# ZhaozhiQIAN/Hybrid-ODE-NeurIPS-2021

Hardware: AMD Instinct MI355X
Metric: patient-trajectories/sec (fwd+adjoint) at dim=12, T=100 (higher is better)
Workload: dtype f32; 1 GPU; dim12 synthetic, 10000 patients/GPU, T=100, dt=0.125, rk4(3/8), fused rhs+step kernel + discrete-adjoint kernel (split expert/learned wave pipelines); patients_total=10000, launch=hipGraph, lanes_per_patient=auto, theta_grad=True, parallelism=dp1, n_ranks=1, stage_tape=True

## Files before the change

### hybrid-ode-neurips-2021_amd/csrc/hode_rk_split.hip

```cpp
#include <hip/hip_runtime.h>
#include <stdlib.h>

#include "../../include/hode.h"
#include "hode_common.hpp"
#include "hode_host.hpp"
#include "hode_roche.hpp"

namespace hode {

#ifndef HODE_SPLIT_EXPERT_FIRST
#define HODE_SPLIT_EXPERT_FIRST 1
#endif
constexpr int kSplitPatients = 48;

struct SplitArgs {
  const float* __restrict__ t;
  const float* __restrict__ y0;
  const float* __restrict__ dosage;
  const float* __restrict__ dose_times;
  const float* __restrict__ theta;
  const float* __restrict__ w1;
  const float* __restrict__ b1;
  float* __restrict__ h;
  float* __restrict__ tape;
  unsigned long long* dbg;
  float* __restrict__ ltape;
  int* __restrict__ status;
  int B, T, K, perturb;
};

struct SpTimes {
  float t0, t1, dt, ts[4];
  HODE_DEV SpTimes(const float* __restrict__ t, int n, int perturb, int method) {
    t0 = t[n];
    t1 = t[n + 1];
    dt = t1 - t0;
    ts[0] = perturb ? nextafter_up(t0) : t0;
    ts[3] = perturb ? nextafter_down(t1) : t1;
    if (method == HODE_METHOD_RK4_38) {
      ts[1] = add_rn(t0, mul_rn(dt, (float)(1.0 / 3.0)));
      ts[2] = add_rn(t0, mul_rn(dt, (float)(2.0 / 3.0)));
    } else {
      ts[1] = add_rn(t0, mul_rn(0.5f, dt));
      ts[2] = ts[1];
    }
  }
};

template <int METHOD>
HODE_DEV float sp_stage_time(float t0, float t1, int perturb, int q) {
  const float dt = t1 - t0;
  const float c = METHOD == HODE_METHOD_RK4_38 ? (q == 1 ? (float)(1.0 / 3.0) : (q == 2 ? (float)(2.0 / 3.0) : 0.f))
                                               : (q == 0 ? 0.f : 0.5f);
  float tq = add_rn(t0, mul_rn(dt, c));
  tq = q == 3 ? t1 : tq;
  if (perturb) {
    if (q == 0) tq = nextafter_up(t0);
    if (q == 3) tq = nextafter_down(t1);
  }
  return tq;
}

constexpr int kSplitMaxT = 8192;
HODE_DEV void sp_stage_grid(float* __restrict__ tg, const float* __restrict__ t, int T) {
  for (int i = threadIdx.x; i < T + 3; i += blockDim.x) tg[i] = t[min(i, T - 1)];
}

template <int METHOD>
constexpr int sp_stages() { return METHOD == HODE_METHOD_EULER ? 1 : (METHOD == HODE_METHOD_MIDPOINT ? 2 : 4); }

template <int METHOD, class V>
HODE_DEV V sp_stage_state(int i, V y, float dt, V k1, V k2, V k3) {
  constexpr float c13 = (float)(1.0 / 3.0);
  if constexpr (METHOD == HODE_METHOD_MIDPOINT) return i == 0 ? y : vfma(k1, vsplat<V>(0.5f * dt), y);
  else if constexpr (METHOD == HODE_METHOD_RK4_38) {
    if (i == 0) return y;
    if (i == 1) return vfma(dt * k1, vsplat<V>(c13), y);
    if (i == 2) return vfma(vsplat<V>(dt), vfma(-k1, vsplat<V>(c13), k2), y);
    return vfma(vsplat<V>(dt), (k1 - k2) + k3, y);
  } else return y;
}
template <int METHOD, class V>
HODE_DEV V sp_advance(V y, float dt, V k1, V k2, V k3, V k4) {
  if constexpr (METHOD == HODE_METHOD_EULER) return vfma(vsplat<V>(dt), k1, y);
  else if constexpr (METHOD == HODE_METHOD_MIDPOINT) return vfma(vsplat<V>(dt), k2, y);
  else return vfma((k1 + 3.0f * (k2 + k3)) + k4, vsplat<V>(dt * 0.125f), y);
}

template <int V> struct IC { static constexpr int value = V; };

template <int MR> struct OwnSel { typedef float type; };
template <> struct OwnSel<2> { typedef f2 type; };

template <bool C, class A, class B> struct TypeSel { typedef A type; };
template <class A, class B> struct TypeSel<false, A, B> { typedef B type; };

#ifndef HODE_LTAPE_STAGES
#define HODE_LTAPE_STAGES 2
#endif
constexpr int kLearnedTapeStages = HODE_LTAPE_STAGES;
template <int METHOD> constexpr int sp_ltape_stages() { return METHOD == HODE_METHOD_RK4_38 ? kLearnedTapeStages : 0; }

template <int D>
struct MlRows {
  static constexpr int M = D - 4, MR = M / 4, DP = D / 2, MP = M / 2;
  static constexpr int NW = MR == 2 ? D : DP;
  static constexpr int NU = MR == 2 ? M : MP;
  static constexpr float kTanhScale = 2.885390081777927f;
  typedef typename OwnSel<MR>::type Own;
  typedef typename TypeSel<MR == 2, float, f2>::type Elem;
  struct Stage { Elem v[NW]; };
  struct Gath { Elem v[NU]; };
  f2 wp[NW];
  Own bias;
  HODE_DEV void load(const float* __restrict__ W, const float* __restrict__ b, int q) {
    if constexpr (MR == 2) {
#pragma unroll
      for (int i = 0; i < D; ++i) wp[i] = kTanhScale * pair2(W[(2 * q) * D + i], W[(2 * q + 1) * D + i]);
      bias = kTanhScale * pair2(b[2 * q], b[2 * q + 1]);
    } else {
#pragma unroll
      for (int ip = 0; ip < DP; ++ip) wp[ip] = kTanhScale * pair2(W[q * D + 2 * ip], W[q * D + 2 * ip + 1]);
      bias = kTanhScale * b[q];
    }
  }
  static HODE_DEV void gather(Own v, Elem* __restrict__ out) {
    if constexpr (MR == 2) {
      out[0] = quad_bcast<0>(v.x); out[1] = quad_bcast<0>(v.y);
      out[2] = quad_bcast<1>(v.x); out[3] = quad_bcast<1>(v.y);
      out[4] = quad_bcast<2>(v.x); out[5] = quad_bcast<2>(v.y);
      out[6] = quad_bcast<3>(v.x); out[7] = quad_bcast<3>(v.y);
    } else {
      out[0] = pair2(quad_bcast<0>(v), quad_bcast<1>(v));
      out[1] = pair2(quad_bcast<2>(v), quad_bcast<3>(v));
    }
  }
  static HODE_DEV Stage stage(const float4& e, Own Yo) {
    Stage Y;
    if constexpr (MR == 2) {
      Y.v[0] = e.x; Y.v[1] = e.y; Y.v[2] = e.z; Y.v[3] = e.w;
      gather(Yo, Y.v + 4);
    } else {
      Y.v[0] = pair2(e.x, e.y);
      Y.v[1] = pair2(e.z, e.w);
      gather(Yo, Y.v + 2);
    }
    return Y;
  }
  static HODE_DEV Own tanh_scaled(Own z) {
    if constexpr (MR == 2) {
      const f2 e = pair2(__builtin_amdgcn_exp2f(z.x), __builtin_amdgcn_exp2f(z.y)) + splat2(1.0f);
      return vfma(pair2(__builtin_amdgcn_rcpf(e.x), __builtin_amdgcn_rcpf(e.y)), splat2(-2.0f), splat2(1.0f));
    } else {
      return __builtin_fmaf(__builtin_amdgcn_rcpf(__builtin_amdgcn_exp2f(z) + 1.0f), -2.0f, 1.0f);
    }
  }
  HODE_DEV Own rhs(const Stage& Y) const {
    if constexpr (MR == 2) {
      f2 acc = bias, acc1 = splat2(0.f);
#pragma unroll
      for (int i = 0; i < D; i += 2) {
        acc = vfma(wp[i], Y.v[i], acc);
        acc1 = vfma(wp[i + 1], Y.v[i + 1], acc1);
      }
      return tanh_scaled(acc + acc1);
    } else {
      f2 acc = pair2(bias, 0.f);
#pragma unroll
      for (int ip = 0; ip < DP; ++ip) acc = vfma(wp[ip], Y.v[ip], acc);
      return tanh_scaled(hsum(acc));
    }
  }
  struct Part { f2 a, b; };
  HODE_DEV Part rhs_expert(const float4& e) const {
    Part p;
    if constexpr (MR == 2) {
      p.a = vfma(wp[2], e.z, vfma(wp[0], e.x, bias));
      p.b = vfma(wp[3], e.w, vfma(wp[1], e.y, splat2(0.f)));
    } else {
      p.a = vfma(wp[1], pair2(e.z, e.w), vfma(wp[0], pair2(e.x, e.y), pair2(bias, 0.f)));
      p.b = splat2(0.f);
    }
    return p;
  }
  HODE_DEV Own rhs_rest(const Part& p, const Stage& Y) const {
    if constexpr (MR == 2) {
      f2 acc = p.a, acc1 = p.b;
#pragma unroll
      for (int i = 4; i < D; i += 2) {
        acc = vfma(wp[i], Y.v[i], acc);
        acc1 = vfma(wp[i + 1], Y.v[i + 1], acc1);
      }
      return tanh_scaled(acc + acc1);
    } else {
      f2 acc = p.a;
#pragma unroll
      for (int ip = 2; ip < DP; ++ip) acc = vfma(wp[ip], Y.v[ip], acc);
      return tanh_scaled(hsum(acc));
    }
  }
  static HODE_DEV void outer_acc(f2 (&dw)[NW], Own u, const Stage& Y) {
#pragma unroll
    for (int i = 0; i < NW; ++i) dw[i] = vfma(u, Y.v[i], dw[i]);
  }
  static HODE_DEV float dw_at(const f2 (&dw)[NW], int r, int i) {
    if constexpr (MR == 2) return r == 0 ? dw[i].x : dw[i].y;
    else return (i & 1) ? dw[i / 2].y : dw[i / 2].x;
  }
  static HODE_DEV Own load_own(const float* __restrict__ src, int q) {
    if constexpr (MR == 2) {
      const float2 x = *reinterpret_cast<const float2*>(src + 4 + 2 * q);
      return pair2(x.x, x.y);
    } else return src[4 + q];
  }
  static HODE_DEV void store_own(float* __restrict__ dst, int q, Own v) {
    if constexpr (MR == 2) *reinterpret_cast<float2*>(dst + 4 + 2 * q) = make_float2(v.x, v.y);
    else dst[4 + q] = v;
  }
  template <int NL>
  static HODE_DEV void store_tape(float* __restrict__ dst, const Own* __restrict__ k) {
    if constexpr (MR == 2 && NL % 2 == 0) {
#pragma unroll
      for (int i = 0; i < NL; i += 2)
        *reinterpret_cast<float4*>(dst + 4 * (i / 2)) = make_float4(k[i].x, k[i].y, k[i + 1].x, k[i + 1].y);
    } else if constexpr (MR == 1 && NL == 4) {
      *reinterpret_cast<float4*>(dst) = make_float4(k[0], k[1], k[2], k[3]);
    } else if constexpr (MR == 1 && NL == 2) {
      *reinterpret_cast<float2*>(dst) = make_float2(k[0], k[1]);
    } else {
#pragma unroll
      for (int i = 0; i < NL; ++i) {
        if constexpr (MR == 2) *reinterpret_cast<float2*>(dst + 2 * i) = make_float2(k[i].x, k[i].y);
        else dst[i] = k[i];
      }
    }
  }
  template <int NL>
  static HODE_DEV void load_tape(const float* __restrict__ src, Own* __restrict__ k) {
    if constexpr (MR == 2 && NL % 2 == 0) {
#pragma unroll
      for (int i = 0; i < NL; i += 2) {
        const float4 v = *reinterpret_cast<const float4*>(src + 4 * (i / 2));
        k[i] = pair2(v.x, v.y); k[i + 1] = pair2(v.z, v.w);
      }
    } else if constexpr (MR == 1 && NL == 4) {
      const float4 v = *reinterpret_cast<const float4*>(src);
      k[0] = v.x; k[1] = v.y; k[2] = v.z; k[3] = v.w;
    } else if constexpr (MR == 1 && NL == 2) {
      const float2 v = *reinterpret_cast<const float2*>(src);
      k[0] = v.x; k[1] = v.y;
    } else {
#pragma unroll
      for (int i = 0; i < NL; ++i) {
        if constexpr (MR == 2) { const float2 v = *reinterpret_cast<const float2*>(src + 2 * i); k[i] = pair2(v.x, v.y); }
        else k[i] = src[i];
      }
    }
  }
};

template <int D, int METHOD, bool ABLATE, bool HILL2, bool K1, bool TAPE>
HODE_DEV void split_fwd_body(const SplitArgs& a) {
  constexpr int NS = sp_stages<METHOD>();
  typedef MlRows<D> Ml;
  typedef typename Ml::Own Own;
  constexpr int DP = Ml::DP;
  __shared__ __attribute__((aligned(16))) float ring[2][4][kSplitPatients][4];
  __shared__ __attribute__((aligned(16))) float dring[2][kSplitPatients][4];
  extern __shared__ float tg[];
  const int tid = threadIdx.x;
  const int wave = tid >> 6, lane = tid & 63;
  const int b0 = blockIdx.x * kSplitPatients;
  const RocheTheta th = load_theta(a.theta, ABLATE);
  const size_t row = (size_t)a.B * D;
  sp_stage_grid(tg, a.t, a.T);
#ifdef HODE_SPLIT_STAMPS
#define HODE_FSTAMP(k) if (a.dbg && blockIdx.x == 0 && lane == 0) a.dbg[(size_t)wave * a.T + (k)] = __builtin_amdgcn_s_memtime();
#else
#define HODE_FSTAMP(k)
#endif

  if (wave == 0) {
    const int slot = lane;
    const bool live = slot < kSplitPatients && b0 + slot < a.B;
    const int p = min(b0 + (slot < kSplitPatients ? slot : 0), a.B - 1);
    const int rslot = slot < kSplitPatients ? slot : 0;
    const unsigned lane_h = (unsigned)p * D, lane_t = (unsigned)p * 4;
    MlSlice<4, 1> none;
    float own1[1];
    f2 ya, yb;
    {
      const float4 v = *reinterpret_cast<const float4*>(a.y0 + (size_t)p * D);
      ya = pair2(v.x, v.y);
      yb = pair2(v.z, v.w);
      if (live) *reinterpret_cast<float4*>(a.h + (size_t)p * D) = v;
    }
    __syncthreads();
    auto e_iter = [&](int it, auto PAR) {
      constexpr int par = decltype(PAR)::value;
      if (it + 1 < a.T) {
        const float dt = tg[it + 1] - tg[it];
        const float4 dz = *reinterpret_cast<const float4*>(&dring[par][rslot][0]);
        const float dose[4] = {dz.x, dz.y, dz.z, dz.w};
        float* __restrict__ tape_it = TAPE ? a.tape + (size_t)it * (NS - 1) * a.B * 4 : nullptr;
        f2 ka[4], kb[4];
#pragma unroll
        for (int s = 0; s < 4; ++s) ka[s] = kb[s] = splat2(0.f);
#pragma unroll
        for (int s = 0; s < NS; ++s) {
          const f2 Ya = sp_stage_state<METHOD>(s, ya, dt, ka[0], ka[1], ka[2]);
          const f2 Yb = sp_stage_state<METHOD>(s, yb, dt, kb[0], kb[1], kb[2]);
          if (slot < kSplitPatients) *reinterpret_cast<float4*>(&ring[par][s][slot][0]) = make_float4(Ya.x, Ya.y, Yb.x, Yb.y);
          if constexpr (TAPE) {
            if (s >= 1)
              *reinterpret_cast<float4*>(tape_it + ((unsigned)(s - 1) * (unsigned)a.B * 4u + lane_t)) = make_float4(Ya.x, Ya.y, Yb.x, Yb.y);
          }
          const float Y[4] = {Ya.x, Ya.y, Yb.x, Yb.y};
          float k[4];
          roche_rhs<4, 1, ABLATE, HILL2>(th, none, dose[s], Y, k, own1);
          ka[s] = pair2(k[0], k[1]);
          kb[s] = pair2(k[2], k[3]);
        }
        ya = sp_advance<METHOD>(ya, dt, ka[0], ka[1], ka[2], ka[3]);
        yb = sp_advance<METHOD>(yb, dt, kb[0], kb[1], kb[2], kb[3]);
        *reinterpret_cast<float4*>(a.h + (size_t)(it + 1) * row + lane_h) = make_float4(ya.x, ya.y, yb.x, yb.y);
      }
      HODE_FSTAMP(it)
      __syncthreads();
    };
    for (int it = 0; it < a.T; it += 2) {
      e_iter(it, IC<0>{});
      if (it + 1 < a.T) e_iter(it + 1, IC<1>{});
    }
    if (a.status) {
      const bool bad = !(vfinite(ya) && vfinite(yb));
      if (bad && live) atomicOr(a.status, HODE_STATUS_NONFINITE);
    }
  } else {
    const int q = lane & 3;
    const int slot = (wave - 1) * 16 + (lane >> 2);
    const bool live = b0 + slot < a.B;
    const int p = min(b0 + slot, a.B - 1);
    Ml ml;
    ml.load(a.w1, a.b1, q);
    DoseSched<K1> ds;
    ds.dosage = a.dosage[p];
    ds.K = a.K;
    ds.taus = a.dose_times + (size_t)p * a.K;
    ds.tau0 = K1 ? ds.taus[0] : 0.f;
    auto dose_step = [&](int parity, float t0, float t1) {
      dring[parity][slot][q] = ds.at(sp_stage_time<METHOD>(t0, t1, a.perturb, q), th.kel).v;
    };
    if (a.T >= 2) dose_step(0, a.t[0], a.t[1]);
    if (a.T >= 3) dose_step(1, a.t[1], a.t[2]);
    Own yo = Ml::load_own(a.y0 + (size_t)p * D, q);
    if (live) Ml::store_own(a.h + (size_t)p * D, q, yo);
    constexpr int NLT = sp_ltape_stages<METHOD>();
    const size_t lt_step = (size_t)a.B * 4 * NLT * Ml::MR;
    const unsigned lt_lane = ((unsigned)p * 4 + q) * NLT * Ml::MR;
    __syncthreads();
    __syncthreads();
    auto m_iter = [&](int it, auto PAR) {
      constexpr int par = decltype(PAR)::value;
      const int n = it - 1;
      const float t_a = tg[it - 1], t_b = tg[it], t_c = tg[it + 1], t_d = tg[it + 2];
      const float dt = t_b - t_a;
      Own k[4];
      float4 e[4];
#pragma unroll
      for (int s = 0; s < NS; ++s) e[s] = *reinterpret_cast<const float4*>(&ring[par][s][slot][0]);
      __builtin_amdgcn_sched_barrier(0);
      dose_step(par, t_c, t_d);
#if HODE_SPLIT_EXPERT_FIRST
      typename Ml::Part pe[4];
#pragma unroll
      for (int s = 0; s < NS; ++s) pe[s] = ml.rhs_expert(e[s]);
#endif
#pragma unroll
      for (int s = 0; s < 4; ++s) k[s] = vsplat<Own>(0.f);
#pragma unroll
      for (int s = 0; s < NS; ++s) {
        const Own Yo = sp_stage_state<METHOD>(s, yo, dt, k[0], k[1], k[2]);
#if HODE_SPLIT_EXPERT_FIRST
        k[s] = ml.rhs_rest(pe[s], Ml::stage(e[s], Yo));
#else
        k[s] = ml.rhs(Ml::stage(e[s], Yo));
#endif
      }
      yo = sp_advance<METHOD>(yo, dt, k[0], k[1], k[2], k[3]);
      Ml::store_own(a.h + (size_t)(n + 1) * row + (size_t)p * D, q, yo);
      if constexpr (TAPE && NLT > 0) Ml::template store_tape<NLT>(a.ltape + (size_t)n * lt_step + lt_lane, k + (NS - NLT));
      HODE_FSTAMP(it)
      __syncthreads();
    };
    for (int it = 1; it < a.T; it += 2) {
      m_iter(it, IC<0>{});
      if (it + 1 < a.T) m_iter(it + 1, IC<1>{});
    }
    if (a.status) {
      if (!vfinite(yo) && live) atomicOr(a.status, HODE_STATUS_NONFINITE);
    }
  }
}

struct SplitBwdArgs {
  const float* __restrict__ t;
  const float* __restrict__ dosage;
  const float* __restrict__ dose_times;
  const float* __restrict__ theta;
  const float* __restrict__ w1;
  const float* __restrict__ b1;
  const float* __restrict__ h;
  const float* __restrict__ grad_h;
  float* __restrict__ grad_y0;
  float* __restrict__ part_ml;
  float* __restrict__ part_th;
  const float* __restrict__ tape;
  const float* __restrict__ ltape;
  int B, T, K, perturb;
  unsigned long long* dbg;
};

template <int METHOD, class V, class F>
HODE_DEV void sp_adjoint_step(V& lam, float dt, F&& vjp) {
  constexpr float c13 = (float)(1.0 / 3.0);
  if constexpr (METHOD == HODE_METHOD_EULER) {
    lam += vjp(0, dt * lam);
  } else if constexpr (METHOD == HODE_METHOD_MIDPOINT) {
    const V a1 = vjp(1, dt * lam);
    lam += a1;
    lam += vjp(0, (0.5f * dt) * a1);
  } else {
    const float w1 = dt * 0.125f, w3 = dt * 0.375f;
    const V a3 = vjp(3, w1 * lam);
    V da = dt * a3;
    V g1 = vfma(w1, lam, da);
    V g2 = vfma(w3, lam, -da);
    const V g = vfma(w3, lam, da);
    lam += a3;
    const V a2 = vjp(2, g);
    da = dt * a2;
    g2 += da;
    g1 = vfma(-c13, da, g1);
    lam += a2;
    const V a1 = vjp(1, g2);
    g1 = vfma(c13, dt * a1, g1);
    lam += a1;
    lam += vjp(0, g1);
  }
}

struct F4 {
  f2 a, b;
  HODE_DEV F4& operator+=(const F4& o) { a += o.a; b += o.b; return *this; }
  HODE_DEV F4 operator-() const { return F4{-a, -b}; }
};
HODE_DEV F4 operator*(float s, const F4& v) { return F4{s * v.a, s * v.b}; }
HODE_DEV F4 vfma(float s, const F4& x, const F4& y) { return F4{vfma(s, x.a, y.a), vfma(s, x.b, y.b)}; }

template <int D, bool CW>
struct SplitBwdShared {
  static constexpr int RD = CW ? 3 : 2;
  static constexpr int M = D - 4;
  float yring[RD][4][kSplitPatients][4];
  float cring[RD][4][kSplitPatients + 1][4];
  float dring[RD][kSplitPatients][8];
  float gring[RD][4][kSplitPatients + 1][4];
  float tdring[RD][kSplitPatients][8];
  float uring[CW ? RD : 1][4][CW ? kSplitPatients : 1][CW ? M : 1];
  float red[4][4][M * D + M];
};

template <int D, int METHOD, bool ABLATE, bool HILL2, bool NEED_TH, bool K1, bool TAPE>
HODE_DEV void split_bwd_body(const SplitBwdArgs& a, SplitBwdShared<D, TAPE>& sh) {
  constexpr int NS = sp_stages<METHOD>();
  typedef MlRows<D> Ml;
  typedef typename Ml::Own Own;
  constexpr int M = Ml::M, MR = Ml::MR, DP = Ml::DP, MP = Ml::MP;
  constexpr bool THW = TAPE && NEED_TH;
  constexpr bool CW = TAPE;
  constexpr int RD = SplitBwdShared<D, TAPE>::RD;
  constexpr int EL = CW ? 2 : 1;
  constexpr int CWAVE = THW ? 5 : 4;
  auto& yring = sh.yring; auto& cring = sh.cring; auto& dring = sh.dring; auto& gring = sh.gring;
  auto& tdring = sh.tdring; auto& uring = sh.uring; auto& red = sh.red;
  extern __shared__ float tg[];
  const int tid = threadIdx.x;
  const int wave = tid >> 6, lane = tid & 63;
  const int b0 = blockIdx.x * kSplitPatients;
  const RocheTheta th = load_theta(a.theta, ABLATE);
  const size_t row = (size_t)a.B * D;
  const int T = a.T;
  const int NIT = T + EL - 1;
  sp_stage_grid(tg, a.t, a.T);
#ifdef HODE_SPLIT_STAMPS
#define HODE_SSTAMP(k) if (a.dbg && blockIdx.x == 0 && lane == 0) a.dbg[(size_t)wave * (a.T + 2) + (k)] = __builtin_amdgcn_s_memtime();
#define HODE_PSTAMP(k, ph) { __builtin_amdgcn_sched_barrier(0); if (a.dbg && blockIdx.x == 0 && wave == 3 && lane == 0) a.dbg[(size_t)6 * (a.T + 2) + 64 + (size_t)(k) * 8 + (ph)] = __builtin_amdgcn_s_memtime(); __builtin_amdgcn_sched_barrier(0); }
  if (a.dbg && blockIdx.x < 8 && lane == 0) a.dbg[(size_t)6 * (a.T + 2) + blockIdx.x * 8 + wave] = __builtin_amdgcn_s_getreg(63492);
#else
#define HODE_SSTAMP(k)
#define HODE_PSTAMP(k, ph)
#endif
  auto run = [&](auto&& iter) {
    for (int k = 0; k < NIT; k += RD) {
      iter(k, IC<0>{});
      if (k + 1 < NIT) iter(k + 1, IC<1>{});
      if constexpr (RD == 3) {
        if (k + 2 < NIT) iter(k + 2, IC<2>{});
      }
    }
  };

  if (wave == 0) {
    const int slot = lane < kSplitPatients ? lane : 0;
    const bool mine = lane < kSplitPatients;
    const bool live = mine && b0 + slot < a.B;
    const int p = min(b0 + slot, a.B - 1);
    const float lv = live ? 1.0f : 0.0f;
    DoseSched<K1> ds;
    ds.dosage = a.dosage[p];
    ds.K = a.K;
    ds.taus = a.dose_times + (size_t)p * a.K;
    ds.tau0 = K1 ? ds.taus[0] : 0.f;
    const float ln_ec50 = log_f32(th.ec50);
    const int cslot = mine ? lane : kSplitPatients;
    if (lane < 16 * RD) (&cring[lane >> 4][(lane >> 2) & 3][kSplitPatients][0])[lane & 3] = 0.f;
    const unsigned lane_h = (unsigned)p * D, lane_t = (unsigned)p * 4;
    MlSlice<4, 1> none;
    MlColSlice<4, 1> nonec;
    GradAcc<4, 1> acc;
    acc.zero();
    float own1[1] = {0.f};

    float tp[4][4];
    auto fetch = [&](int m) {
      const float4 v = *reinterpret_cast<const float4*>(a.h + (size_t)m * row + lane_h);
      tp[0][0] = v.x; tp[0][1] = v.y; tp[0][2] = v.z; tp[0][3] = v.w;
      if constexpr (TAPE) {
        const float* __restrict__ tape_m = a.tape + (size_t)m * (NS - 1) * a.B * 4;
#pragma unroll
        for (int s = 1; s < NS; ++s) {
          const float4 u = *reinterpret_cast<const float4*>(tape_m + ((unsigned)(s - 1) * (unsigned)a.B * 4u + lane_t));
          tp[s][0] = u.x; tp[s][1] = u.y; tp[s][2] = u.z; tp[s][3] = u.w;
        }
      }
    };
    auto publish = [&](int m, int par) {
      if constexpr (TAPE) {
        if (mine) {
#pragma unroll
          for (int s = 0; s < NS; ++s)
            *reinterpret_cast<float4*>(&yring[par][s][slot][0]) = make_float4(tp[s][0], tp[s][1], tp[s][2], tp[s][3]);
        }
      } else {
        const SpTimes st(a.t, m, a.perturb, METHOD);
        const f2 ya = pair2(tp[0][0], tp[0][1]), yb = pair2(tp[0][2], tp[0][3]);
        f2 ka[4], kb[4];
#pragma unroll
        for (int s = 0; s < 4; ++s) ka[s] = kb[s] = splat2(0.f);
#pragma unroll
        for (int s = 0; s < NS; ++s) {
          const f2 Ya = sp_stage_state<METHOD>(s, ya, st.dt, ka[0], ka[1], ka[2]);
          const f2 Yb = sp_stage_state<METHOD>(s, yb, st.dt, kb[0], kb[1], kb[2]);
          const DoseVal dv = ds.at(st.ts[s], th.kel);
          if (mine) {
            *reinterpret_cast<float4*>(&yring[par][s][slot][0]) = make_float4(Ya.x, Ya.y, Yb.x, Yb.y);
            dring[par][slot][s] = dv.v;
            dring[par][slot][4 + s] = dv.dk;
          }
          if (s + 1 < NS) {
            const float Y[4] = {Ya.x, Ya.y, Yb.x, Yb.y};
            float k[4];
            roche_rhs<4, 1, ABLATE, HILL2>(th, none, dv.v, Y, k, own1);
            ka[s] = pair2(k[0], k[1]);
            kb[s] = pair2(k[2], k[3]);
          }
        }
      }
    };

    F4 lam;
    {
      const float4 g4 = *reinterpret_cast<const float4*>(a.grad_h + (size_t)(T - 1) * row + (size_t)p * D);
      lam.a = lv * pair2(g4.x, g4.y);
      lam.b = lv * pair2(g4.z, g4.w);
    }
    if (T >= 2) {
      fetch(T - 2);
      publish(T - 2, 0);
    }
    __syncthreads();
    auto e_iter = [&](int k, auto SI) {
      constexpr int S = decltype(SI)::value;
      constexpr int par = (S + 1) % RD;
      if (T - 3 - k >= 0) fetch(T - 3 - k);
      if (k >= EL && k <= T + EL - 2) {
        const int m = T - k + EL - 2;
        const float dt = tg[m + 1] - tg[m];
        float Y[4][4];
        F4 cs[4];
        DoseVal dv[4];
        {
          const float4 d0 = *reinterpret_cast<const float4*>(&dring[par][slot][0]);
          const float4 d1 = *reinterpret_cast<const float4*>(&dring[par][slot][4]);
          dv[0].v = d0.x; dv[1].v = d0.y; dv[2].v = d0.z; dv[3].v = d0.w;
          dv[0].dk = d1.x; dv[1].dk = d1.y; dv[2].dk = d1.z; dv[3].dk = d1.w;
          if constexpr (THW) {
            *reinterpret_cast<float4*>(&tdring[S][slot][0]) = d0;
            *reinterpret_cast<float4*>(&tdring[S][slot][4]) = d1;
          }
        }
#pragma unroll
        for (int s = 0; s < NS; ++s) {
          const float4 yv = *reinterpret_cast<const float4*>(&yring[par][s][slot][0]);
          const float4 cv = *reinterpret_cast<const float4*>(&cring[par][s][cslot][0]);
          Y[s][0] = yv.x; Y[s][1] = yv.y; Y[s][2] = yv.z; Y[s][3] = yv.w;
          cs[s].a = pair2(cv.x, cv.y);
          cs[s].b = pair2(cv.z, cv.w);
        }
        sp_adjoint_step<METHOD>(lam, dt, [&](int s, const F4& gs) {
          const float g[4] = {gs.a.x, gs.a.y, gs.b.x, gs.b.y};
          float av[4];
          if constexpr (THW) {
            if (mine) *reinterpret_cast<float4*>(&gring[S][s][slot][0]) = make_float4(g[0], g[1], g[2], g[3]);
          }
          roche_vjp<4, 1, ABLATE, HILL2, NEED_TH && !THW>(th, none, nonec, ln_ec50, dv[s], Y[s], own1, g, 0, av, acc);
          F4 r = cs[s];
          r.a += pair2(av[0], av[1]);
          r.b += pair2(av[2], av[3]);
          return r;
        });
        const float4 g4 = *reinterpret_cast<const float4*>(a.grad_h + (size_t)m * row + lane_h);
        lam.a = vfma(lv, pair2(g4.x, g4.y), lam.a);
        lam.b = vfma(lv, pair2(g4.z, g4.w), lam.b);
      }
      if (T - 3 - k >= 0) publish(T - 3 - k, par);
      HODE_SSTAMP(k)
      __syncthreads();
    };
    run(e_iter);
    if (live) *reinterpret_cast<float4*>(a.grad_y0 + (size_t)p * D) = make_float4(lam.a.x, lam.a.y, lam.b.x, lam.b.y);
    if constexpr (!THW) {
#pragma unroll
      for (int i = 0; i < kNTheta; ++i) {
        const float v = row_sum(NEED_TH ? acc.dth[i] : 0.f);
        if ((lane & 15) == 0) red[0][lane >> 4][i] = v;
      }
      __builtin_amdgcn_fence(__ATOMIC_SEQ_CST, "wavefront");
      if (lane < kNTheta)
        a.part_th[(size_t)blockIdx.x * kNTheta + lane] = (red[0][0][lane] + red[0][1][lane]) + (red[0][2][lane] + red[0][3][lane]);
    }
  } else if (THW && wave == 4) {
    const int slot = lane < kSplitPatients ? lane : 0;
    const bool mine = lane < kSplitPatients;
    const int p = min(b0 + slot, a.B - 1);
    const int gslot = mine ? lane : kSplitPatients;
    const float ln_ec50 = log_f32(th.ec50);
    if (lane < 16 * RD) (&gring[lane >> 4][(lane >> 2) & 3][kSplitPatients][0])[lane & 3] = 0.f;
    const unsigned lane_h = (unsigned)p * D, lane_t = (unsigned)p * 4;
    float dth[kNTheta];
#pragma unroll
    for (int i = 0; i < kNTheta; ++i) dth[i] = 0.f;
    float tp[4][4];
    auto fetch = [&](int m) {
      const float4 v = *reinterpret_cast<const float4*>(a.h + (size_t)m * row + lane_h);
      tp[0][0] = v.x; tp[0][1] = v.y; tp[0][2] = v.z; tp[0][3] = v.w;
      const float* __restrict__ tape_m = a.tape + (size_t)m * (NS - 1) * a.B * 4;
#pragma unroll
      for (int s = 1; s < NS; ++s) {
        const float4 u = *reinterpret_cast<const float4*>(tape_m + ((unsigned)(s - 1) * (unsigned)a.B * 4u + lane_t));
        tp[s][0] = u.x; tp[s][1] = u.y; tp[s][2] = u.z; tp[s][3] = u.w;
      }
    };
    auto theta_step = [&](int gpar) {
      const float4 d0 = *reinterpret_cast<const float4*>(&tdring[gpar][slot][0]);
      const float4 d1 = *reinterpret_cast<const float4*>(&tdring[gpar][slot][4]);
      const float dvv[4] = {d0.x, d0.y, d0.z, d0.w}, dvk[4] = {d1.x, d1.y, d1.z, d1.w};
#pragma unroll
      for (int si = 0; si < NS; ++si) {
        const int s = NS - 1 - si;
        const float4 gv = *reinterpret_cast<const float4*>(&gring[gpar][s][gslot][0]);
        DoseVal dv;
        dv.v = dvv[s]; dv.dk = dvk[s];
        const float g[4] = {gv.x, gv.y, gv.z, gv.w};
        roche_theta_grad<ABLATE, HILL2>(th, ln_ec50, dv, tp[s], g, dth);
      }
    };
    __syncthreads();
    auto t_iter = [&](int k, auto SI) {
      constexpr int S = decltype(SI)::value;
      constexpr int gpar = (S + RD - 1) % RD;
      if (k >= EL + 1) theta_step(gpar);
      if (k >= EL && T - k + EL - 2 >= 0) fetch(T - k + EL - 2);
      HODE_SSTAMP(k)
      __syncthreads();
    };
    run(t_iter);
    if (T >= 2) theta_step((NIT - 1) % RD);
#pragma unroll
    for (int i = 0; i < kNTheta; ++i) {
      const float v = row_sum(dth[i]);
      if ((lane & 15) == 0) red[0][lane >> 4][i] = v;
    }
    __builtin_amdgcn_fence(__ATOMIC_SEQ_CST, "wavefront");
    if (lane < kNTheta)
      a.part_th[(size_t)blockIdx.x * kNTheta + lane] = (red[0][0][lane] + red[0][1][lane]) + (red[0][2][lane] + red[0][3][lane]);
  } else if (CW && wave == CWAVE) {
    const int slot = lane < kSplitPatients ? lane : 0;
    const bool mine = lane < kSplitPatients;
    float wq[M][4];
#pragma unroll
    for (int j = 0; j < M; ++j)
#pragma unroll
      for (int q = 0; q < 4; ++q) wq[j][q] = a.w1[j * D + q];
    __syncthreads();
    auto c_iter = [&](int k, auto SI) {
      constexpr int S = decltype(SI)::value;
      constexpr int cpar = (S + RD - 1) % RD;
      if (k >= 1 && k - 1 <= T - 2) {
        float u[NS][M];
#pragma unroll
        for (int s = 0; s < NS; ++s) {
#pragma unroll
          for (int j4 = 0; j4 < M; j4 += 4) {
            const float4 v = *reinterpret_cast<const float4*>(&uring[cpar][s][slot][j4]);
            u[s][j4] = v.x; u[s][j4 + 1] = v.y; u[s][j4 + 2] = v.z; u[s][j4 + 3] = v.w;
          }
        }
        __builtin_amdgcn_sched_barrier(0);
#pragma unroll
        for (int s = 0; s < NS; ++s) {
          float c[4];
#pragma unroll
          for (int q = 0; q < 4; ++q) {
            if constexpr (MR == 2) {
              float cq = 0.f;
#pragma unroll
              for (int j = 0; j < M; ++j) cq = __builtin_fmaf(wq[j][q], u[s][j], cq);
              c[q] = cq;
            } else {
              float cx = 0.f, cy = 0.f;
#pragma unroll
              for (int jp = 0; jp < MP; ++jp) {
                cx = __builtin_fmaf(wq[2 * jp][q], u[s][2 * jp], cx);
                cy = __builtin_fmaf(wq[2 * jp + 1][q], u[s][2 * jp + 1], cy);
              }
              c[q] = cx + cy;
            }
          }
          if (mine) *reinterpret_cast<float4*>(&cring[cpar][s][slot][0]) = make_float4(c[0], c[1], c[2], c[3]);
        }
      }
      HODE_SSTAMP(k)
      __syncthreads();
    };
    run(c_iter);
  } else {
    const int q = lane & 3;
    const int slot = (wave - 1) * 16 + (lane >> 2);
    const bool live = b0 + slot < a.B;
    const int p = min(b0 + slot, a.B - 1);
    const float lv = live ? 1.0f : 0.0f;
    Ml ml;
    ml.load(a.w1, a.b1, q);
    typename Ml::Elem wc[Ml::NU];
    f2 wtp[Ml::NU];
    if constexpr (MR == 2) {
#pragma unroll
      for (int j = 0; j < M; ++j) {
        wc[j] = a.w1[j * D + q];
        wtp[j] = pair2(a.w1[j * D + 4 + 2 * q], a.w1[j * D + 4 + 2 * q + 1]);
      }
    } else {
#pragma unroll
      for (int jp = 0; jp < MP; ++jp) {
        wc[jp] = pair2(a.w1[(2 * jp) * D + q], a.w1[(2 * jp + 1) * D + q]);
        wtp[jp] = pair2(a.w1[(2 * jp) * D + 4 + q], a.w1[(2 * jp + 1) * D + 4 + q]);
      }
    }
    f2 dw[Ml::NW];
    Own db = vsplat<Own>(0.f);
#pragma unroll
    for (int i = 0; i < Ml::NW; ++i) dw[i] = splat2(0.f);
    DoseSched<K1> ds;
    ds.dosage = a.dosage[p];
    ds.K = a.K;
    ds.taus = a.dose_times + (size_t)p * a.K;
    ds.tau0 = K1 ? ds.taus[0] : 0.f;
    Own lam = lv * Ml::load_own(a.grad_h + (size_t)(T - 1) * row + (size_t)p * D, q);
    Own yo_nx, gh_nx;
    constexpr int NLT = TAPE ? sp_ltape_stages<METHOD>() : 0;
    const size_t lt_step = (size_t)a.B * 4 * NLT * MR;
    const unsigned lt_lane = ((unsigned)p * 4 + q) * NLT * MR;
    Own lt_nx[NLT > 0 ? NLT : 1], lt_n2[NLT > 0 ? NLT : 1];
    {
      const int m0 = T >= 2 ? T - 2 : 0;
      const int m1 = m0 >= 1 ? m0 - 1 : 0;
      yo_nx = Ml::load_own(a.h + (size_t)m0 * row + (size_t)p * D, q);
      gh_nx = Ml::load_own(a.grad_h + (size_t)m0 * row + (size_t)p * D, q);
      if constexpr (NLT > 0) {
        Ml::template load_tape<NLT>(a.ltape + (size_t)m0 * lt_step + lt_lane, lt_nx);
        Ml::template load_tape<NLT>(a.ltape + (size_t)m1 * lt_step + lt_lane, lt_n2);
      }
    }
    __syncthreads();
    auto m_iter = [&](int k, auto SI) {
      constexpr int par = decltype(SI)::value;
      if (k <= T - 2) {
        HODE_PSTAMP(k, 0)
        const int m = T - 2 - k;
        const float t0 = tg[m], t1 = tg[m + 1];
        const float dt = t1 - t0;
        const Own yo = yo_nx, gh = gh_nx;
        Own lt[NLT > 0 ? NLT : 1];
#pragma unroll
        for (int i = 0; i < NLT; ++i) { lt[i] = lt_nx[i]; lt_nx[i] = lt_n2[i]; }
        {
          const int mn = m >= 1 ? m - 1 : 0;
          yo_nx = Ml::load_own(a.h + (size_t)mn * row + (size_t)p * D, q);
          gh_nx = Ml::load_own(a.grad_h + (size_t)mn * row + (size_t)p * D, q);
          if constexpr (NLT > 0) Ml::template load_tape<NLT>(a.ltape + (size_t)(m >= 2 ? m - 2 : 0) * lt_step + lt_lane, lt_n2);
        }
        typename Ml::Stage Y[4];
        Own so[4];
        float4 e[4];
#pragma unroll
        for (int s = 0; s < NS; ++s) e[s] = *reinterpret_cast<const float4*>(&yring[par][s][slot][0]);
        __builtin_amdgcn_sched_barrier(0);
        HODE_PSTAMP(k, 1)
        if constexpr (TAPE) {
          const DoseVal dq = ds.at(sp_stage_time<METHOD>(t0, t1, a.perturb, q), th.kel);
          dring[par][slot][q] = dq.v;
          if constexpr (NEED_TH) dring[par][slot][4 + q] = dq.dk;
        }
#if HODE_SPLIT_EXPERT_FIRST
        typename Ml::Part pe[4];
#pragma unroll
        for (int s = 0; s < NS - NLT; ++s) pe[s] = ml.rhs_expert(e[s]);
#endif
#pragma unroll
        for (int s = 0; s < 4; ++s) so[s] = vsplat<Own>(0.f);
#pragma unroll
        for (int s = 0; s < NS; ++s) {
          const Own Yo = sp_stage_state<METHOD>(s, yo, dt, so[0], so[1], so[2]);
          Y[s] = Ml::stage(e[s], Yo);
          if (s >= NS - NLT) so[s] = lt[s - (NS - NLT) < 0 ? 0 : s - (NS - NLT)];
#if HODE_SPLIT_EXPERT_FIRST
          else so[s] = ml.rhs_rest(pe[s], Y[s]);
#else
          else so[s] = ml.rhs(Y[s]);
#endif
        }
        HODE_PSTAMP(k, 2)
        sp_adjoint_step<METHOD>(lam, dt, [&](int s, Own gs) {
          HODE_PSTAMP(k, 6 - s)
          const Own u = gs * vfma(-so[s], so[s], vsplat<Own>(1.0f));
          db += u;
          Ml::outer_acc(dw, u, Y[s]);
          if constexpr (CW) {
            if constexpr (MR == 2) *reinterpret_cast<float2*>(&uring[par][s][slot][2 * q]) = make_float2(u.x, u.y);
            else uring[par][s][slot][q] = u;
          }
          typename Ml::Gath uf;
          Ml::gather(u, uf.v);
          if constexpr (MR == 2) {
            float cq = 0.f;
            f2 av = splat2(0.f), av1 = splat2(0.f);
#pragma unroll
            for (int j = 0; j < M; j += 2) {
              if constexpr (!CW) cq = __builtin_fmaf(wc[j], uf.v[j], cq);
              av = vfma(wtp[j], uf.v[j], av);
              if constexpr (!CW) cq = __builtin_fmaf(wc[j + 1], uf.v[j + 1], cq);
              av1 = vfma(wtp[j + 1], uf.v[j + 1], av1);
            }
            if constexpr (!CW) cring[par][s][slot][q] = cq;
            return av + av1;
          } else {
            f2 c2 = splat2(0.f), a2 = splat2(0.f);
#pragma unroll
            for (int jp = 0; jp < MP; ++jp) {
              if constexpr (!CW) c2 = vfma(wc[jp], uf.v[jp], c2);
              a2 = vfma(wtp[jp], uf.v[jp], a2);
            }
            if constexpr (!CW) cring[par][s][slot][q] = hsum(c2);
            return hsum(a2);
          }
        });
        lam = vfma(lv, gh, lam);
        HODE_PSTAMP(k, 7)
      }
      HODE_SSTAMP(k)
      __syncthreads();
    };
    run(m_iter);
    if (live) Ml::store_own(a.grad_y0 + (size_t)p * D, q, lam);
    float* out = a.part_ml + ((size_t)blockIdx.x * 3 + (wave - 1)) * (M * D + M);
    const bool writer = (lane & 15) < 4;
    float* mine = &red[wave][lane >> 4][0];
#pragma unroll
    for (int r = 0; r < MR; ++r) {
#pragma unroll
      for (int i = 0; i < D; ++i) {
        const float v = row_sum_stride4(Ml::dw_at(dw, r, i));
        if (writer) mine[(q * MR + r) * D + i] = v;
      }
      float dbr;
      if constexpr (MR == 2) dbr = r == 0 ? db.x : db.y;
      else dbr = db;
      const float vb = row_sum_stride4(dbr);
      if (writer) mine[M * D + q * MR + r] = vb;
    }
    __builtin_amdgcn_fence(__ATOMIC_SEQ_CST, "wavefront");
    for (int c = lane; c < M * D + M; c += 64)
      out[c] = (red[wave][0][c] + red[wave][1][c]) + (red[wave][2][c] + red[wave][3][c]);
  }
}

__global__ __launch_bounds__(64) void split_fold_kernel(const float* __restrict__ part_ml, const float* __restrict__ part_th,
                                                        int nblk, int P_ml, int n_w, float* __restrict__ gw,
                                                        float* __restrict__ gb, float* __restrict__ gth, int need_th,
                                                        int overwrite) {
  const int j = blockIdx.x;
  const int lane = threadIdx.x;
  const bool ml = j < P_ml;
  const float* src = ml ? part_ml + j : part_th + (j - P_ml);
  const int rows = ml ? 3 * nblk : nblk;
  const int stride = ml ? P_ml : kNTheta;
  float s = 0.f;
  for (int base = 0; base < rows; base += 64 * 8) {
    float v[8];
#pragma unroll
    for (int q = 0; q < 8; ++q) {
      const int w = base + lane + 64 * q;
      v[q] = w < rows ? src[(size_t)w * stride] : 0.f;
    }
#pragma unroll
    for (int q = 0; q < 8; ++q) s += v[q];
  }
  s = wave_sum(s);
  if (lane != 0) return;
  float* dst = nullptr;
  if (ml) dst = j < n_w ? (gw ? gw + j : nullptr) : (gb ? gb + (j - n_w) : nullptr);
  else if (gth) dst = gth + (j - P_ml);
  if (!dst) return;
  if (!ml && !need_th) s = 0.f;
  *dst = overwrite ? s : *dst + s;
}

#ifndef HODE_SPLIT_WPE_FWD
#define HODE_SPLIT_WPE_FWD 2
#endif
#ifndef HODE_SPLIT_WPE_BWD
#define HODE_SPLIT_WPE_BWD 2
#endif
#ifndef HODE_SPLIT_WPE_BWD_MIN
#define HODE_SPLIT_WPE_BWD_MIN 1
#endif

template <int D, int METHOD, bool ABLATE, bool NEED_TH, bool TAPE>
__global__ __launch_bounds__(384) __attribute__((amdgpu_waves_per_eu(HODE_SPLIT_WPE_BWD_MIN, HODE_SPLIT_WPE_BWD))) void split_bwd_kernel(SplitBwdArgs a) {
  __shared__ __attribute__((aligned(16))) SplitBwdShared<D, TAPE> sh;
  const bool hill2 = ABLATE || (a.theta[0] == 2.0f && a.theta[1] == 2.0f);
  if (hill2 && a.K == 1) split_bwd_body<D, METHOD, ABLATE, true, NEED_TH, true, TAPE>(a, sh);
  else if (hill2) split_bwd_body<D, METHOD, ABLATE, true, NEED_TH, false, TAPE>(a, sh);
  else split_bwd_body<D, METHOD, ABLATE, false, NEED_TH, false, TAPE>(a, sh);
}

template <int D, int METHOD, bool ABLATE, bool TAPE>
__global__ __launch_bounds__(256) __attribute__((amdgpu_waves_per_eu(1, HODE_SPLIT_WPE_FWD))) void split_fwd_kernel(SplitArgs a) {
  const bool hill2 = ABLATE || (a.theta[0] == 2.0f && a.theta[1] == 2.0f);
  if (hill2 && a.K == 1) split_fwd_body<D, METHOD, ABLATE, true, true, TAPE>(a);
  else if (hill2) split_fwd_body<D, METHOD, ABLATE, true, false, TAPE>(a);
  else split_fwd_body<D, METHOD, ABLATE, false, false, TAPE>(a);
}

}

namespace {

template <int D, bool ABLATE>
int split_method(const hode_solve_desc* d, const hode::SplitArgs& a, hipStream_t s) {
  const dim3 grid((d->batch + hode::kSplitPatients - 1) / hode::kSplitPatients), block(256);
  const size_t lds = (size_t)(d->n_times + 3) * sizeof(float);
#define HODE_SPLIT_FWD(M)                                                                                 \
  if (a.tape) hipLaunchKernelGGL((hode::split_fwd_kernel<D, M, ABLATE, true>), grid, block, lds, s, a);   \
  else hipLaunchKernelGGL((hode::split_fwd_kernel<D, M, ABLATE, false>), grid, block, lds, s, a);
  switch (d->method) {
    case HODE_METHOD_EULER: HODE_SPLIT_FWD(HODE_METHOD_EULER) break;
    case HODE_METHOD_MIDPOINT: HODE_SPLIT_FWD(HODE_METHOD_MIDPOINT) break;
    default: HODE_SPLIT_FWD(HODE_METHOD_RK4_38) break;
  }
  return hode::hip_fail(hipGetLastError(), "split kernel launch");
}

}

namespace {

template <int D, bool ABLATE>
int split_bwd_method(const hode_solve_desc* d, const hode::SplitBwdArgs& a, hipStream_t s) {
  const dim3 grid((d->batch + hode::kSplitPatients - 1) / hode::kSplitPatients), block(256);
  const size_t lds = (size_t)(d->n_times + 3) * sizeof(float);
#define HODE_SPLIT_BWD(M)                                                                                        \
  if (d->need_theta_grad) {                                                                                      \
    if (a.tape) hipLaunchKernelGGL((hode::split_bwd_kernel<D, M, ABLATE, true, true>), grid, dim3(384), lds, s, a); \
    else hipLaunchKernelGGL((hode::split_bwd_kernel<D, M, ABLATE, true, false>), grid, block, lds, s, a);          \
  } else {                                                                                                       \
    if (a.tape) hipLaunchKernelGGL((hode::split_bwd_kernel<D, M, ABLATE, false, true>), grid, dim3(320), lds, s, a); \
    else hipLaunchKernelGGL((hode::split_bwd_kernel<D, M, ABLATE, false, false>), grid, block, lds, s, a);         \
  }
  switch (d->method) {
    case HODE_METHOD_EULER: HODE_SPLIT_BWD(HODE_METHOD_EULER) break;
    case HODE_METHOD_MIDPOINT: HODE_SPLIT_BWD(HODE_METHOD_MIDPOINT) break;
    default: HODE_SPLIT_BWD(HODE_METHOD_RK4_38) break;
  }
  return hode::hip_fail(hipGetLastError(), "split bwd kernel launch");
}

}

namespace hode {

bool split_supported(const hode_solve_desc* d) { return (d->latent_dim == 8 || d->latent_dim == 12) && d->n_times <= kSplitMaxT; }

static size_t al256s(size_t x) { return (x + 255) / 256 * 256; }

static int n_stages(int method) { return method == HODE_METHOD_EULER ? 1 : (method == HODE_METHOD_MIDPOINT ? 2 : 4); }

static size_t split_partials_bytes(const hode_solve_desc* d) {
  const size_t nblk = (d->batch + kSplitPatients - 1) / kSplitPatients;
  const size_t M = d->latent_dim - 4;
  return al256s(nblk * 3 * (M * d->latent_dim + M) * sizeof(float)) + al256s(nblk * kNTheta * sizeof(float));
}
static size_t split_etape_bytes(const hode_solve_desc* d) {
  if (!(d->flags & HODE_FLAG_TAPE) || d->n_times < 2) return 0;
  return al256s((size_t)(d->n_times - 1) * (n_stages(d->method) - 1) * d->batch * 4 * sizeof(float));
}
static size_t split_ltape_bytes(const hode_solve_desc* d) {
  if (!(d->flags & HODE_FLAG_TAPE) || d->n_times < 2 || n_stages(d->method) != 4 || kLearnedTapeStages == 0) return 0;
  return al256s((size_t)(d->n_times - 1) * d->batch * (d->latent_dim - 4) * kLearnedTapeStages * sizeof(float));
}
static size_t split_tape_bytes(const hode_solve_desc* d) { return split_etape_bytes(d) + split_ltape_bytes(d); }
size_t split_workspace_bytes(const hode_solve_desc* d) { return split_partials_bytes(d) + split_tape_bytes(d); }
static float* split_tape(const hode_solve_desc* d) {
  return split_etape_bytes(d) ? (float*)((char*)d->workspace + split_partials_bytes(d)) : nullptr;
}
static float* split_ltape(const hode_solve_desc* d) {
  return split_ltape_bytes(d) ? (float*)((char*)d->workspace + split_partials_bytes(d) + split_etape_bytes(d)) : nullptr;
}

int split_rk_bwd(const hode_solve_desc* d, hipStream_t s) {
  const int nblk = (d->batch + kSplitPatients - 1) / kSplitPatients;
  const int M = d->latent_dim - 4;
  const int Pml = M * d->latent_dim + M;
  char* ws = (char*)d->workspace;
  SplitBwdArgs a{};
  a.t = d->t; a.dosage = d->dosage; a.dose_times = d->dose_times; a.theta = d->theta; a.w1 = d->w1; a.b1 = d->b1;
  a.h = d->h; a.grad_h = d->grad_h; a.grad_y0 = d->grad_y0;
  a.part_ml = (float*)ws;
  a.part_th = (float*)(ws + al256s((size_t)nblk * 3 * Pml * sizeof(float)));
  a.B = d->batch; a.T = d->n_times; a.K = d->n_dose; a.perturb = d->perturb;
  a.tape = split_tape(d);
  a.ltape = split_ltape(d);
#ifdef HODE_SPLIT_STAMPS
  if (const char* env = getenv("HODE_SPLIT_DBG_PTR")) a.dbg = (unsigned long long*)strtoull(env, nullptr, 0);
#endif
  const bool abl = d->rhs_kind == HODE_RHS_ROCHE_ABLATE;
  int e;
  if (d->latent_dim == 8) e = abl ? split_bwd_method<8, true>(d, a, s) : split_bwd_method<8, false>(d, a, s);
  else e = abl ? split_bwd_method<12, true>(d, a, s) : split_bwd_method<12, false>(d, a, s);
  if (e || (d->flags & HODE_FLAG_SKIP_FOLD)) return e;
  const bool th_out = d->grad_theta != nullptr && (d->need_theta_grad || (d->flags & HODE_FLAG_OVERWRITE_GRADS));
  hipLaunchKernelGGL(split_fold_kernel, dim3(Pml + (th_out ? kNTheta : 0)), dim3(64), 0, s, a.part_ml, a.part_th, nblk, Pml,
                     M * d->latent_dim, d->grad_w1, d->grad_b1, d->grad_theta, d->need_theta_grad,
                     (d->flags & HODE_FLAG_OVERWRITE_GRADS) ? 1 : 0);
  return hip_fail(hipGetLastError(), "split_fold launch");
}

int split_rk_fwd(const hode_solve_desc* d, hipStream_t s) {
  SplitArgs a{};
  a.t = d->t; a.y0 = d->y0; a.dosage = d->dosage; a.dose_times = d->dose_times; a.theta = d->theta; a.w1 = d->w1; a.b1 = d->b1;
  a.h = d->h; a.status = d->status;
  a.B = d->batch; a.T = d->n_times; a.K = d->n_dose; a.perturb = d->perturb;
  a.tape = split_tape(d);
  a.ltape = split_ltape(d);
#ifdef HODE_SPLIT_STAMPS
  if (const char* env = getenv("HODE_SPLIT_FWD_DBG_PTR")) a.dbg = (unsigned long long*)strtoull(env, nullptr, 0);
#endif
  const bool abl = d->rhs_kind == HODE_RHS_ROCHE_ABLATE;
  if (d->latent_dim == 8) return abl ? split_method<8, true>(d, a, s) : split_method<8, false>(d, a, s);
  return abl ? split_method<12, true>(d, a, s) : split_method<12, false>(d, a, s);
}

}
```

Measured before the change: 75.88 million trajectories/s.

## Restructure split-adjoint LDS rings to cut bank conflicts and shrink footprint

Reorganizes the shared-memory rings of the split backward kernel. dring and tdring become planar [2][patients][4], and uring is split into float4 column groups laid out per patient. Idle lanes now map to distinct slots and zero rows instead of all aliasing slot 0, and cring is unioned with the reduction buffer to cut LDS usage. The aim is fewer LDS bank conflicts and broadcasts on the wave rings, and possibly higher occupancy. The union relies on red and cring never being live at the same time.

```diff
diff --git a/hybrid-ode-neurips-2021_amd/csrc/hode_rk_split.hip b/hybrid-ode-neurips-2021_amd/csrc/hode_rk_split.hip
--- a/hybrid-ode-neurips-2021_amd/csrc/hode_rk_split.hip
+++ b/hybrid-ode-neurips-2021_amd/csrc/hode_rk_split.hip
@@ -458,18 +458,29 @@
 HODE_DEV F4 operator*(float s, const F4& v) { return F4{s * v.a, s * v.b}; }
 HODE_DEV F4 vfma(float s, const F4& x, const F4& y) { return F4{vfma(s, x.a, y.a), vfma(s, x.b, y.b)}; }
 
+constexpr int kSplitZeroRowA = kSplitPatients, kSplitZeroRowB = kSplitPatients + 4;
+constexpr int kSplitCRows = kSplitZeroRowB + 1;
+constexpr int kSplitURows = kSplitPatients + 4;
+HODE_DEV int sp_lane_slot(int lane) { return lane < kSplitPatients ? lane : lane - 16; }
+HODE_DEV int sp_zero_row(int lane) { return lane >= 52 && lane < 60 ? kSplitZeroRowB : kSplitZeroRowA; }
+
 template <int D, bool CW>
 struct SplitBwdShared {
   static constexpr int RD = CW ? 3 : 2;
   static constexpr int M = D - 4;
+  static constexpr int UP = M / 4;
   float yring[RD][4][kSplitPatients][4];
-  float cring[RD][4][kSplitPatients + 1][4];
-  float dring[RD][kSplitPatients][8];
-  float gring[RD][4][kSplitPatients + 1][4];
-  float tdring[RD][kSplitPatients][8];
-  float uring[CW ? RD : 1][4][CW ? kSplitPatients : 1][CW ? M : 1];
-  float red[4][4][M * D + M];
+  union {
+    float cring[RD][4][kSplitCRows][4];
+    float red[4][4][M * D + M];
+  };
+  float dring[RD][2][kSplitPatients][4];
+  float gring[RD][4][kSplitCRows][4];
+  float tdring[RD][2][kSplitPatients][4];
+  float uring[CW ? RD : 1][4][CW ? UP : 1][CW ? kSplitURows : 1][4];
 };
+static_assert(sizeof(SplitBwdShared<12, false>::cring) >= sizeof(SplitBwdShared<12, false>::red) &&
+              sizeof(SplitBwdShared<8, false>::cring) >= sizeof(SplitBwdShared<8, false>::red), "red takes cring's place");
 
 template <int D, int METHOD, bool ABLATE, bool HILL2, bool NEED_TH, bool K1, bool TAPE>
 HODE_DEV void split_bwd_body(const SplitBwdArgs& a, SplitBwdShared<D, TAPE>& sh) {
@@ -512,7 +523,7 @@
   };
 
   if (wave == 0) {
-    const int slot = lane < kSplitPatients ? lane : 0;
+    const int slot = sp_lane_slot(lane);
     const bool mine = lane < kSplitPatients;
     const bool live = mine && b0 + slot < a.B;
     const int p = min(b0 + slot, a.B - 1);
@@ -523,8 +534,11 @@
     ds.taus = a.dose_times + (size_t)p * a.K;
     ds.tau0 = K1 ? ds.taus[0] : 0.f;
     const float ln_ec50 = log_f32(th.ec50);
-    const int cslot = mine ? lane : kSplitPatients;
-    if (lane < 16 * RD) (&cring[lane >> 4][(lane >> 2) & 3][kSplitPatients][0])[lane & 3] = 0.f;
+    const int cslot = mine ? lane : sp_zero_row(lane);
+    if (lane < 16 * RD) {
+      (&cring[lane >> 4][(lane >> 2) & 3][kSplitZeroRowA][0])[lane & 3] = 0.f;
+      (&cring[lane >> 4][(lane >> 2) & 3][kSplitZeroRowB][0])[lane & 3] = 0.f;
+    }
     const unsigned lane_h = (unsigned)p * D, lane_t = (unsigned)p * 4;
     MlSlice<4, 1> none;
     MlColSlice<4, 1> nonec;
@@ -565,8 +579,8 @@
           const DoseVal dv = ds.at(st.ts[s], th.kel);
           if (mine) {
             *reinterpret_cast<float4*>(&yring[par][s][slot][0]) = make_float4(Ya.x, Ya.y, Yb.x, Yb.y);
-            dring[par][slot][s] = dv.v;
-            dring[par][slot][4 + s] = dv.dk;
+            dring[par][0][slot][s] = dv.v;
+            dring[par][1][slot][s] = dv.dk;
           }
           if (s + 1 < NS) {
             const float Y[4] = {Ya.x, Ya.y, Yb.x, Yb.y};
@@ -601,13 +615,13 @@
         F4 cs[4];
         DoseVal dv[4];
         {
-          const float4 d0 = *reinterpret_cast<const float4*>(&dring[par][slot][0]);
-          const float4 d1 = *reinterpret_cast<const float4*>(&dring[par][slot][4]);
+          const float4 d0 = *reinterpret_cast<const float4*>(&dring[par][0][slot][0]);
+          const float4 d1 = *reinterpret_cast<const float4*>(&dring[par][1][slot][0]);
           dv[0].v = d0.x; dv[1].v = d0.y; dv[2].v = d0.z; dv[3].v = d0.w;
           dv[0].dk = d1.x; dv[1].dk = d1.y; dv[2].dk = d1.z; dv[3].dk = d1.w;
           if constexpr (THW) {
-            *reinterpret_cast<float4*>(&tdring[S][slot][0]) = d0;
-            *reinterpret_cast<float4*>(&tdring[S][slot][4]) = d1;
+            *reinterpret_cast<float4*>(&tdring[S][0][slot][0]) = d0;
+            *reinterpret_cast<float4*>(&tdring[S][1][slot][0]) = d1;
           }
         }
 #pragma unroll
@@ -651,30 +665,33 @@
         a.part_th[(size_t)blockIdx.x * kNTheta + lane] = (red[0][0][lane] + red[0][1][lane]) + (red[0][2][lane] + red[0][3][lane]);
     }
   } else if (THW && wave == 4) {
-    const int slot = lane < kSplitPatients ? lane : 0;
+    const int slot = sp_lane_slot(lane);
     const bool mine = lane < kSplitPatients;
     const int p = min(b0 + slot, a.B - 1);
-    const int gslot = mine ? lane : kSplitPatients;
+    const int gslot = mine ? lane : sp_zero_row(lane);
     const float ln_ec50 = log_f32(th.ec50);
-    if (lane < 16 * RD) (&gring[lane >> 4][(lane >> 2) & 3][kSplitPatients][0])[lane & 3] = 0.f;
+    if (lane < 16 * RD) {
+      (&gring[lane >> 4][(lane >> 2) & 3][kSplitZeroRowA][0])[lane & 3] = 0.f;
+      (&gring[lane >> 4][(lane >> 2) & 3][kSplitZeroRowB][0])[lane & 3] = 0.f;
+    }
     const unsigned lane_h = (unsigned)p * D, lane_t = (unsigned)p * 4;
     float dth[kNTheta];
 #pragma unroll
     for (int i = 0; i < kNTheta; ++i) dth[i] = 0.f;
     float tp[4][4];
-    auto fetch = [&](int m) {
+    auto fetch = [&](int m, float (&dst)[4][4]) {
       const float4 v = *reinterpret_cast<const float4*>(a.h + (size_t)m * row + lane_h);
-      tp[0][0] = v.x; tp[0][1] = v.y; tp[0][2] = v.z; tp[0][3] = v.w;
+      dst[0][0] = v.x; dst[0][1] = v.y; dst[0][2] = v.z; dst[0][3] = v.w;
       const float* __restrict__ tape_m = a.tape + (size_t)m * (NS - 1) * a.B * 4;
 #pragma unroll
       for (int s = 1; s < NS; ++s) {
         const float4 u = *reinterpret_cast<const float4*>(tape_m + ((unsigned)(s - 1) * (unsigned)a.B * 4u + lane_t));
-        tp[s][0] = u.x; tp[s][1] = u.y; tp[s][2] = u.z; tp[s][3] = u.w;
+        dst[s][0] = u.x; dst[s][1] = u.y; dst[s][2] = u.z; dst[s][3] = u.w;
       }
     };
     auto theta_step = [&](int gpar) {
-      const float4 d0 = *reinterpret_cast<const float4*>(&tdring[gpar][slot][0]);
-      const float4 d1 = *reinterpret_cast<const float4*>(&tdring[gpar][slot][4]);
+      const float4 d0 = *reinterpret_cast<const float4*>(&tdring[gpar][0][slot][0]);
+      const float4 d1 = *reinterpret_cast<const float4*>(&tdring[gpar][1][slot][0]);
       const float dvv[4] = {d0.x, d0.y, d0.z, d0.w}, dvk[4] = {d1.x, d1.y, d1.z, d1.w};
 #pragma unroll
       for (int si = 0; si < NS; ++si) {
@@ -691,7 +708,7 @@
       constexpr int S = decltype(SI)::value;
       constexpr int gpar = (S + RD - 1) % RD;
       if (k >= EL + 1) theta_step(gpar);
-      if (k >= EL && T - k + EL - 2 >= 0) fetch(T - k + EL - 2);
+      if (k >= EL && T - k + EL - 2 >= 0) fetch(T - k + EL - 2, tp);
       HODE_SSTAMP(k)
       __syncthreads();
     };
@@ -706,7 +723,7 @@
     if (lane < kNTheta)
       a.part_th[(size_t)blockIdx.x * kNTheta + lane] = (red[0][0][lane] + red[0][1][lane]) + (red[0][2][lane] + red[0][3][lane]);
   } else if (CW && wave == CWAVE) {
-    const int slot = lane < kSplitPatients ? lane : 0;
+    const int slot = sp_lane_slot(lane);
     const bool mine = lane < kSplitPatients;
     float wq[M][4];
 #pragma unroll
@@ -723,7 +740,7 @@
         for (int s = 0; s < NS; ++s) {
 #pragma unroll
           for (int j4 = 0; j4 < M; j4 += 4) {
-            const float4 v = *reinterpret_cast<const float4*>(&uring[cpar][s][slot][j4]);
+            const float4 v = *reinterpret_cast<const float4*>(&uring[cpar][s][j4 / 4][slot][0]);
             u[s][j4] = v.x; u[s][j4 + 1] = v.y; u[s][j4 + 2] = v.z; u[s][j4 + 3] = v.w;
           }
         }
@@ -830,8 +847,8 @@
         HODE_PSTAMP(k, 1)
         if constexpr (TAPE) {
           const DoseVal dq = ds.at(sp_stage_time<METHOD>(t0, t1, a.perturb, q), th.kel);
-          dring[par][slot][q] = dq.v;
-          if constexpr (NEED_TH) dring[par][slot][4 + q] = dq.dk;
+          dring[par][0][slot][q] = dq.v;
+          if constexpr (NEED_TH) dring[par][1][slot][q] = dq.dk;
         }
 #if HODE_SPLIT_EXPERT_FIRST
         typename Ml::Part pe[4];
@@ -858,8 +875,8 @@
           db += u;
           Ml::outer_acc(dw, u, Y[s]);
           if constexpr (CW) {
-            if constexpr (MR == 2) *reinterpret_cast<float2*>(&uring[par][s][slot][2 * q]) = make_float2(u.x, u.y);
-            else uring[par][s][slot][q] = u;
+            if constexpr (MR == 2) *reinterpret_cast<float2*>(&uring[par][s][q >> 1][slot][2 * (q & 1)]) = make_float2(u.x, u.y);
+            else uring[par][s][0][slot][q] = u;
           }
           typename Ml::Gath uf;
           Ml::gather(u, uf.v);
```

Result: no change. 76.42 million trajectories/s (median of 6 runs) (+0.7%).
